# chanzuckerberg/shasta

Hardware: NVIDIA H100
Metric: candidate_pairs_found_and_aligned_per_s (higher is better)
Workload: dtype u64/i32

## Files before the change

shasta_b200/csrc/align.cu:

```cuda
#include "context.cuh"
#include "align_kernels.cuh"
#include "hostpool.cuh"
#include "digest.cuh"

#include <algorithm>
#include <atomic>
#include <exception>
#include <memory>
#include <mutex>
#include <chrono>
#include <cstring>
#include <sys/mman.h>
#include <thread>
#include <limits>
#include <map>
#include <vector>

namespace shb {

extern thread_local uint64_t g_launchCount;

namespace {

uint32_t warpsForClass(const DpClass& k)
{
    if(k.c > 0) return kDpMaxWarpsPerBlock;
    const uint64_t perWarp = 3ull * (k.wMax + 1) * 4;
    const uint32_t w = uint32_t(std::min<uint64_t>(kDpMaxWarpsPerBlock, (200ull * 1024) / perWarp));
    return w ? w : 1;
}
size_t smemForClass(const DpClass& k, uint32_t warps) { return k.c > 0 ? 0 : size_t(warps) * 3 * (k.wMax + 1) * 4; }
size_t scanKernelSmemLimit()
{
    size_t most = 0;
    for(uint32_t k = 0; k < kDpClassCount; k++) most = std::max(most, smemForClass(dpClassAt(k), warpsForClass(dpClassAt(k))));
// ... 207 lines not shown
    const uint32_t rows = uint32_t(2 * c->readCountTotal);
    sc.sortedKmer.reserve(M + 1);
    sc.sortedOrdinal.reserve(M + 1);
    const std::vector<uint64_t>& toc = c->tocHost;
    DeviceBuffer<uint64_t> keysA, keysB;
    DeviceBuffer<uint32_t> valsA, valsB;
    const uint64_t chunkLimit = envCount("SHB_ALIGN4_SORT_CHUNK", 1u << 28);
    uint32_t rowBegin = 0;
    while(rowBegin < rows) {
        uint32_t rowEnd = rowBegin + 1;
        while(rowEnd < rows && toc[rowEnd + 1] - toc[rowBegin] <= chunkLimit) rowEnd++;
        const uint64_t markerBegin = toc[rowBegin];
        const uint64_t n64 = toc[rowEnd] - markerBegin;
        SHB_REQUIRE(n64 < (1ull << 32), SHB_ERR_INVALID, "An oriented read has more than 2^32-1 markers.");
        const uint32_t n = uint32_t(n64);
        if(n) {
            keysA.reserve(n); keysB.reserve(n); valsA.reserve(n); valsB.reserve(n);
            SHB_LAUNCH(sortedMarkerKeysKernel, ceilDiv(n, 256), 256, 0, st, c->kmerIds, (const uint64_t*)c->toc.get(),
                       rowBegin, rowEnd, markerBegin, n, keysA.get(), valsA.get());
            const uint32_t rowBits = bitsFor(rowEnd - rowBegin - 1);
            const int ranges[2][2] = {{0, int(2 * k)}, {32, 32 + int(rowBits)}};
            const bool inB = radixSort<true>(keysA.get(), keysB.get(), valsA.get(), valsB.get(), n, ranges, 2, c->sortWs, st);
            SHB_LAUNCH(sortedMarkerUnpackKernel, ceilDiv(n, 256), 256, 0, st, (const uint64_t*)(inB ? keysB.get() : keysA.get()), n,
                       sc.sortedKmer.get() + markerBegin);
            SHB_CUDA(cudaMemcpyAsync(sc.sortedOrdinal.get() + markerBegin, inB ? valsB.get() : valsA.get(), 4ull * n,
                                     cudaMemcpyDeviceToDevice, st));
        }
        rowBegin = rowEnd;
    }
    SHB_CUDA(cudaStreamSynchronize(st));
    sc.sortedGeneration = c->markerGeneration;
}

void parallelMemcpy(uint8_t* dst, const uint8_t* src, uint64_t n)
{
    constexpr int kThreads = 4;
    if(n < (4ull << 20)) { memcpy(dst, src, n); return; }
    std::thread workers[kThreads - 1];
    const uint64_t part = (n / kThreads + 4095) & ~4095ull;
    for(int t = 1; t < kThreads; t++) {
        const uint64_t off = std::min<uint64_t>(n, part * t), len = std::min<uint64_t>(part, n - off);
        workers[t - 1] = std::thread([=] { if(len) memcpy(dst + off, src + off, len); });
    }
    memcpy(dst, src, std::min<uint64_t>(part, n));
    for(int t = 1; t < kThreads; t++) workers[t - 1].join();
}

void copyToHostPipelined(shb_context* c, void* dstHost, const void* srcDevice, uint64_t bytes, bool pageLocked)
{
    if(bytes == 0) return;
    if(pageLocked) {
        SHB_CUDA(cudaMemcpyAsync(dstHost, srcDevice, bytes, cudaMemcpyDeviceToHost, c->stream));
        return;
    }
    constexpr uint64_t kChunk = 32ull << 20;
    if(!c->pinnedStage[0]) {
        SHB_CUDA(cudaHostAlloc(&c->pinnedStage[0], kChunk, cudaHostAllocDefault));
        SHB_CUDA(cudaHostAlloc(&c->pinnedStage[1], kChunk, cudaHostAllocDefault));
        SHB_CUDA(cudaEventCreateWithFlags(&c->stageEvent[0], cudaEventDisableTiming));
        SHB_CUDA(cudaEventCreateWithFlags(&c->stageEvent[1], cudaEventDisableTiming));
    }
    cudaStream_t st = c->stream;
    const uint64_t chunks = (bytes + kChunk - 1) / kChunk;
    for(uint64_t k = 0; k <= chunks; k++) {
        if(k < chunks) {
            const uint64_t off = k * kChunk, n = std::min(kChunk, bytes - off);
            SHB_CUDA(cudaMemcpyAsync(c->pinnedStage[k & 1], static_cast<const uint8_t*>(srcDevice) + off, n, cudaMemcpyDeviceToHost, st));
            SHB_CUDA(cudaEventRecord(c->stageEvent[k & 1], st));
        }
        if(k > 0) {
            const uint64_t j = k - 1, off = j * kChunk, n = std::min(kChunk, bytes - off);
            SHB_CUDA(cudaEventSynchronize(c->stageEvent[j & 1]));
            parallelMemcpy(static_cast<uint8_t*>(dstHost) + off, static_cast<const uint8_t*>(c->pinnedStage[j & 1]), n);
        }
    }
}

void buildClassOrder(AlignWorker& w, const DpJob* jobs, uint32_t nJobs, std::vector<uint64_t>& classCounts, bool forward = false)
{
    cudaStream_t st = w.stream;
    Batch& b = w.batch;
    classCounts.assign(kDpClassCount + (forward ? kDpForwardClassCount : 0), 0);
    if(nJobs == 0) return;
    b.orderKeysA.reserve(nJobs); b.orderKeysB.reserve(nJobs); b.orderValsA.reserve(nJobs); b.orderValsB.reserve(nJobs);
    SHB_LAUNCH(dpClassKeysKernel, ceilDiv(nJobs, 256), 256, 0, st, jobs, nJobs, forward, b.orderKeysA.get(), b.orderValsA.get());
    const int ranges[1][2] = {{0, kDpLengthKeyBits + kDpClassKeyBits}};
    const bool inB = radixSort<true>(b.orderKeysA.get(), b.orderKeysB.get(), b.orderValsA.get(), b.orderValsB.get(), nJobs, ranges, 1, w.sortWs, st);
    b.order = inB ? b.orderValsB.get() : b.orderValsA.get();
    unsigned long long* dCounts = w.sc(kScDigits);
    SHB_CUDA(cudaMemsetAsync(dCounts, 0, 256 * sizeof(unsigned long long), st));
    SHB_LAUNCH(digitCountKernel, ceilDiv(nJobs, 256), 256, 0, st, (const uint64_t*)(inB ? b.orderKeysB.get() : b.orderKeysA.get()), nJobs, kDpLengthKeyBits, kDpClassNone, dCounts);
    unsigned long long h[256];
    SHB_CUDA(cudaMemcpyAsync(h, dCounts, sizeof(h), cudaMemcpyDeviceToHost, st));
    SHB_CUDA(cudaStreamSynchronize(st));
    for(size_t k = 0; k < classCounts.size(); k++) classCounts[k] = h[k];
}

template<class F> void runDpClasses(AlignWorker& w, const std::vector<uint64_t>& classCounts, uint32_t chunkMax, uint32_t firstBanded,
                                    const DpJob* jobs, const uint32_t* sequences, DpScores scores, F launchOther)
{
    Batch& b = w.batch;
    BandedArgs g;
    g.kmerIds = sequences; g.scores = scores; g.fma = FmaUnits{1, 2, 4};
    size_t unit = 0;
    forEachClassConcurrently(w, classCounts, chunkMax, [&](int k, uint32_t count, uint64_t offset, cudaStream_t s) {
        const uint32_t* order = b.order + offset;
        if(uint32_t(k) < firstBanded) { launchOther(uint32_t(k), count, order, s); return; }
        const uint32_t cls = uint32_t(k) - firstBanded;
        BandedArgs gk = g;
        gk.n = count; gk.order = order; gk.wMax = dpClassAt(cls).wMax;
// ... 33 lines not shown
    b.ordinals.reserve(ordinalSlots + 1);
    b.runs.reserve(ordinalSlots + 1);
    w.traceWords += traceWords;
    SHB_LAUNCH(setTraceOffsetsKernel, ceilDiv(nJobs, 256), 256, 0, st, b.jobs.get(), nJobs, (const unsigned long long*)b.twOff.get(),
               (const unsigned long long*)b.outOff.get());
    SHB_LAUNCH(bandCellsKernel, ceilDiv(nJobs, 256), 256, 0, st, (const DpJob*)b.jobs.get(), nJobs, w.sc(kScBandCells));
    SHB_CUDA(cudaMemsetAsync(b.counts.get(), 0, 4ull * nJobs, st));
    std::vector<uint64_t> classCounts;
    buildClassOrder(w, b.jobs.get(), nJobs, classCounts);
    SHB_CUDA(cudaEventRecord(w.dp2a, st));
    runDpClasses(w, classCounts, envCount("SHB_ALIGN_CHUNK", 32768), 0, b.jobs.get(), sequences, scores,
                 [](uint32_t, uint32_t, const uint32_t*, cudaStream_t) {});
    SHB_CUDA(cudaEventRecord(w.dp2b, st));
}

struct AlignCall {
    shb_context* c;
    AlignCache* ac;
    const uint32_t* cand; uint64_t n;
    shb_align_options o;
    bool method4;
    DpScores scores; FilterOptions fo;
    uint32_t batchMax;
    uint32_t align4SmemCells = kAlign4SmemCells;
    std::mutex dispenserMutex;
    uint64_t nextBegin = 0, nextIndex = 0;
    struct Segment { uint64_t recordBase = 0, kept = 0, byteBase = 0, bytes = 0; };
    std::mutex arenaMutex;
    std::map<uint64_t, Segment> ledger;
    uint64_t outCount = 0, outBytes = 0;
    cudaStream_t finalStream = nullptr;
    unsigned long long* digests = nullptr;
    uint64_t nextToFinalise = 0, finalRecords = 0, finalBytes = 0;
    uint8_t* hostRecords = nullptr; uint8_t* hostToc = nullptr; uint8_t* hostData = nullptr;
    uint64_t hostDataCapacity = 0;
    bool dataOverflow = false;
    std::atomic<bool> failed{false};
    std::exception_ptr error;
    std::mutex errorMutex;
};

bool nextBatch(AlignCall& call, uint64_t& begin, uint32_t& nb, uint64_t& index)
{
    std::lock_guard<std::mutex> lock(call.dispenserMutex);
    if(call.nextBegin >= call.n || call.failed.load()) return false;
    begin = call.nextBegin;
    nb = 0;
    if(call.method4) {
        const std::vector<uint64_t>& toc = call.c->tocHost;
        const uint64_t cellBudget = 768ull << 20;
        uint64_t cells = 0;
        while(begin + nb < call.n && nb < call.batchMax) {
            const uint64_t i = begin + nb;
            const uint64_t o0 = 2ull * call.cand[3*i], o1 = 2ull * call.cand[3*i+1] + ((call.cand[3*i+2] & 0xff) ? 0 : 1);
            const uint64_t nx = toc[o0+1] - toc[o0], ny = toc[o1+1] - toc[o1];
            uint64_t cc = 2;
            if(nx && ny) cc += ((nx + ny - 2) / call.o.align4DeltaX + 1) * ((nx + ny - 2) / call.o.align4DeltaY + 1);
            if(nb && cells + cc > cellBudget) break;
            cells += cc; nb++;
        }
    } else nb = uint32_t(std::min<uint64_t>(call.batchMax, call.n - begin));
    index = call.nextIndex++;
    call.nextBegin += nb;
    return true;
}

__global__ void rebaseTocKernel(unsigned long long* __restrict__ toc, uint64_t n, long long delta)
{
    const uint64_t i = uint64_t(blockIdx.x) * blockDim.x + threadIdx.x;
    if(i < n) toc[i] = (unsigned long long)((long long)toc[i] + delta);
}

void finaliseReadySegments(AlignCall& call)
{
    AlignCache& ac = *call.ac;
    cudaStream_t fs = call.finalStream;
    for(;;) {
        auto it = call.ledger.find(call.nextToFinalise);
        if(it == call.ledger.end()) break;
        const AlignCall::Segment& seg = it->second;
        if(seg.kept) {
            unsigned long long* segToc = ac.outToc.get() + seg.recordBase;
            const long long delta = (long long)call.finalBytes - (long long)seg.byteBase;
            if(delta) SHB_LAUNCH(rebaseTocKernel, ceilDiv(seg.kept, 256), 256, 0, fs, segToc, seg.kept, delta);
            SHB_LAUNCH(digestRecordsKernel, ceilDiv(seg.kept, 256), 256, 0, fs, (const uint32_t*)ac.outRecords.get() + 16 * seg.recordBase,
                       seg.kept, 16u, call.digests);
            SHB_LAUNCH(digestCompressedKernel, ceilDiv(seg.kept, 256), 256, 0, fs, (const uint32_t*)ac.outRecords.get() + 16 * seg.recordBase,
                       seg.kept, (const unsigned long long*)segToc, call.finalBytes + seg.bytes,
                       (const uint8_t*)ac.outData.get() + seg.byteBase - call.finalBytes, call.digests + 1);
            if(call.hostRecords) {
                SHB_CUDA(cudaMemcpyAsync(call.hostRecords + 64 * call.finalRecords, ac.outRecords.get() + 16 * seg.recordBase, 64 * seg.kept, cudaMemcpyDeviceToHost, fs));
                SHB_CUDA(cudaMemcpyAsync(call.hostToc + 8 * call.finalRecords, segToc, 8 * seg.kept, cudaMemcpyDeviceToHost, fs));
                if(!call.dataOverflow && call.finalBytes + seg.bytes <= call.hostDataCapacity) {
                    SHB_CUDA(cudaMemcpyAsync(call.hostData + call.finalBytes, ac.outData.get() + seg.byteBase, seg.bytes, cudaMemcpyDeviceToHost, fs));
                } else call.dataOverflow = true;
            }
            call.finalRecords += seg.kept; call.finalBytes += seg.bytes;
        }
        call.nextToFinalise++;
    }
}

void processBatch(AlignCall& call, AlignWorker& w, uint64_t begin, uint32_t nb, uint64_t batchIndex)
{
    shb_context* c = call.c;
    AlignCache& ac = *call.ac;
    const shb_align_options& o = call.o;
    cudaStream_t st = w.stream;
    Batch& b = w.batch;
    unsigned long long* total64 = w.sc(kScTotal64);
    uint32_t* total32 = reinterpret_cast<uint32_t*>(w.sc(kScTotal32));

    b.cand.reserve(3ull * nb);
    SHB_CUDA(cudaMemcpyAsync(b.cand.get(), call.cand + 3 * begin, 12ull * nb, cudaMemcpyHostToDevice, st));
    b.keep.reserve(nb); b.keepIndex.reserve(nb); b.bytes32.reserve(nb); b.bytes64.reserve(nb); b.bytesOff.reserve(nb);
    b.scanWs64.reserve(scanWorkspaceElements(nb));
    w.scanWs.reserve(scanWorkspaceElements(std::max<uint64_t>(nb, 4096)));
    uint32_t nJobs = 0;
    const uint32_t* jobIndex = nullptr;
    bool stage1Timed = false;

    if(!call.method4) {
        const bool method1 = (o.alignMethod == 1);
        nJobs = nb;
        b.jobs1.reserve(nb); b.jobs.reserve(nb); b.tw.reserve(nb); b.twOff.reserve(nb); b.outCnt.reserve(nb);
        SHB_LAUNCH(method3SetupKernel, ceilDiv(nb, 256), 256, 0, st, (const uint32_t*)b.cand.get(), nb,
                   (const uint64_t*)c->toc.get(), method1 ? (const uint64_t*)nullptr : (const uint64_t*)ac.dsToc.get(), b.jobs1.get(), b.jobs.get(),
                   b.tw.get(), b.outCnt.get(), w.sc(kScForwardCells), kMaxBandWidth, w.sc(kScTooWide));
        if(!method1) {
// ... 216 lines not shown
                    longest = std::max<uint64_t>(longest, c->tocHost[o + 1] - c->tocHost[o]);
                }
            }
            SHB_REQUIRE(fits(longest), SHB_ERR_INVALID,
                        "Align scores too large for the reads: max(|matchScore|, |mismatchScore|, |gapScore|) * "
                        "(2 * longest read in markers + 16384) must be below 2^28.");
        }
    }
    if(call.method4) {
        SHB_REQUIRE(o.align4DeltaX >= 1 && o.align4DeltaY >= 1 && o.align4DeltaX < (1ull << 31) && o.align4DeltaY < (1ull << 31),
                    SHB_ERR_INVALID, "Invalid Align.align4.deltaX / deltaY.");
        buildSortedMarkers(c, o.k);
    } else if(o.alignMethod == 3) {
        buildDownsampled(c, o.k, o.downsamplingFactor);
    }
    const uint32_t maxStage2Width = uint32_t(std::max(0, o.maxBand)) + 3 + 64;
    SHB_REQUIRE(maxStage2Width <= kMaxBandWidth, SHB_ERR_INVALID, "Align.maxBand too large for this implementation (limit 16317).");

    call.fo.minAlignedMarkerCount = uint64_t(o.minAlignedMarkerCount); call.fo.maxSkip = uint64_t(o.maxSkip);
    call.fo.maxDrift = uint64_t(o.maxDrift); call.fo.maxTrim = uint64_t(o.maxTrim);
    call.fo.minAlignedFraction = o.minAlignedFraction;
    call.fo.suppressContainments = (!call.method4 && o.suppressContainments) ? 1u : 0u;

    call.batchMax = envCount("SHB_ALIGN_BATCH", call.method4 ? 32768 : (o.alignMethod == 1 ? 16384 : 262144));
    call.align4SmemCells = std::min<uint32_t>(kAlign4SmemCells, envCount("SHB_ALIGN4_SMEM_CELLS", kAlign4SmemCells));
    const uint64_t batchEstimate = (n + call.batchMax - 1) / call.batchMax;
    const uint32_t workerCount = uint32_t(std::max<uint64_t>(1, std::min<uint64_t>(envCount("SHB_ALIGN_WORKERS", 2), batchEstimate)));
    while(ac.workers.size() < workerCount) ac.workers.emplace_back(new AlignWorker());
    for(uint32_t k = 0; k < workerCount; k++) ac.workers[k]->init();
    if(!ac.finalStream) SHB_CUDA(cudaStreamCreateWithFlags(&ac.finalStream, cudaStreamNonBlocking));
    call.finalStream = ac.finalStream;
    call.digests = c->scalar(kSlotAlignmentDigests);
    SHB_CUDA(cudaMemsetAsync(call.digests, 0, 2 * sizeof(unsigned long long), st));
    HostResult recOut, tocOut, dataOut;
    if(n && ac.lastBytesPerCandidate > 0.) {
        const uint64_t dataEstimate = uint64_t(ac.lastBytesPerCandidate * double(n) * 1.03) + (1ull << 20);
        recOut.reset(allocHostResult(64 * n)); tocOut.reset(allocHostResult(8 * (n + 1))); dataOut.reset(allocHostResult(dataEstimate));
        if(recOut.p && tocOut.p && dataOut.p && HostPool::instance().isPageLocked(recOut.p) && HostPool::instance().isPageLocked(tocOut.p) &&
           HostPool::instance().isPageLocked(dataOut.p)) {
            call.hostRecords = static_cast<uint8_t*>(recOut.p); call.hostToc = static_cast<uint8_t*>(tocOut.p);
            call.hostData = static_cast<uint8_t*>(dataOut.p); call.hostDataCapacity = dataEstimate;
        }
    }
    SHB_CUDA(cudaStreamSynchronize(st));

    if(n) {
        std::vector<std::thread> threads;
        for(uint32_t k = 0; k < workerCount; k++) threads.emplace_back([&call, &ac, k] { workerMain(call, *ac.workers[k]); });
        for(std::thread& t : threads) t.join();
        if(call.error) std::rethrow_exception(call.error);
    }

    SHB_CUDA(cudaStreamSynchronize(call.finalStream));
    const uint64_t count = call.outCount, outBytes = call.outBytes;
    const auto copy0 = std::chrono::steady_clock::now();
    SHB_REQUIRE(call.nextToFinalise == call.ledger.size() && call.finalRecords == count && call.finalBytes == outBytes, SHB_ERR_CUDA,
                "Internal error: not every batch was finalised.");
    const bool earlyCopy = call.hostRecords != nullptr;
    if(!earlyCopy) {
        recOut.reset(allocHostResult(64 * count)); tocOut.reset(allocHostResult(8 * (count + 1)));
    }
    if(!earlyCopy || call.dataOverflow) dataOut.reset(allocHostResult(outBytes));
    SHB_REQUIRE(recOut.p && tocOut.p && dataOut.p, SHB_ERR_OOM, "Out of host memory for the alignments.");
    if(count && (!earlyCopy || call.dataOverflow)) {
        const bool lockedRec = HostPool::instance().isPageLocked(recOut.p), lockedToc = HostPool::instance().isPageLocked(tocOut.p),
                   lockedData = HostPool::instance().isPageLocked(dataOut.p);
        uint64_t finalRecords = 0, finalBytes = 0;
        for(const auto& entry : call.ledger) {
            const AlignCall::Segment& seg = entry.second;
            if(!seg.kept) continue;
            if(!earlyCopy) {
                copyToHostPipelined(c, static_cast<uint8_t*>(recOut.p) + 64 * finalRecords, ac.outRecords.get() + 16 * seg.recordBase, 64 * seg.kept, lockedRec);
                copyToHostPipelined(c, static_cast<uint8_t*>(tocOut.p) + 8 * finalRecords, ac.outToc.get() + seg.recordBase, 8 * seg.kept, lockedToc);
            }
            copyToHostPipelined(c, static_cast<uint8_t*>(dataOut.p) + finalBytes, ac.outData.get() + seg.byteBase, seg.bytes, lockedData);
            finalRecords += seg.kept; finalBytes += seg.bytes;
        }
        SHB_CUDA(cudaStreamSynchronize(st));
    }
    if(n) ac.lastBytesPerCandidate = double(outBytes) / double(n);
    unsigned long long* digests = call.digests;
    unsigned long long skipped = 0, forwardCells = 0, tooWide = 0, bandCells = 0, digestHost[2] = {0, 0};
    uint64_t traceWords = 0, launches = g_launchCount;
    double dpMs = 0.;
    for(uint32_t k = 0; k < workerCount && n; k++) {
        AlignWorker& w = *ac.workers[k];
        unsigned long long h[6];
        SHB_CUDA(cudaMemcpyAsync(h, w.scalars.get(), sizeof(h), cudaMemcpyDeviceToHost, st));
        SHB_CUDA(cudaStreamSynchronize(st));
        skipped += h[kScSkipped]; forwardCells += h[kScForwardCells]; tooWide += h[kScTooWide]; bandCells += h[kScBandCells];
        traceWords += w.traceWords; launches += w.launches; dpMs += w.dpMs;
    }
    SHB_CUDA(cudaMemcpyAsync(digestHost, digests, sizeof(digestHost), cudaMemcpyDeviceToHost, st));
    SHB_CUDA(cudaStreamSynchronize(st));
    uint64_t* tocHostOut = static_cast<uint64_t*>(tocOut.p);
    tocHostOut[count] = outBytes;
    if(count == 0) tocHostOut[0] = 0;
    totalTimer.stop(st);
    SHB_CUDA(cudaStreamSynchronize(st));
    const float totalMs = totalTimer.elapsedMs();
    if(getenv("SHB_TRACE")) {
        fprintf(stderr, "[shb] computeAlignments: %u worker(s), %llu batches, %llu candidates skipped as too wide for the DP kernels\n",
                workerCount, (unsigned long long)call.ledger.size(), tooWide);
    }
    if(result) {
        memset(result, 0, sizeof(*result));
        result->candidateCount = n; result->alignmentCount = count; result->skippedCount = skipped;
        result->dpCells = 16ull * traceWords + forwardCells;
        result->dpUsefulCells = bandCells + forwardCells;
        result->tooWideCount = tooWide;
        result->dpMs = dpMs / double(workerCount); result->totalMs = totalMs; result->kernelLaunches = launches;
        result->alignmentDataDigest = digestHost[0]; result->compressedDigest = digestHost[1];
        result->workers = workerCount;
        result->outputCopyMs = msSince(copy0);
        result->hostWallMs = msSince(wall0);
    }
    *alignmentDataOut = recOut.take(); *alignmentCountOut = count;
    *compressedTocOut = static_cast<uint64_t*>(tocOut.take()); *compressedDataOut = static_cast<uint8_t*>(dataOut.take());
}

}
```

shasta_b200/csrc/api.cu:

```cuda
#include "context.cuh"
#include <vector>
#include "lowhash_kernels.cuh"
#include "hostpool.cuh"
#include "digest.cuh"

#include <cstring>
#include <string>

namespace shb {

static thread_local std::string g_lastError;
void setLastError(const std::string& message) { g_lastError = message; }

void lowhash0(shb_context* c, const shb_lowhash_params& p, void** candidatesOut, uint64_t* candidateCountOut,
              uint64_t* statsOut, uint64_t* iterSummary, uint64_t maxIterSummary, shb_lowhash_result* result);

void computeAlignments(shb_context* c, const void* candidatesHost, uint64_t n, const shb_align_options& o,
                       void** alignmentDataOut, uint64_t* alignmentCountOut,
                       uint64_t** compressedTocOut, uint8_t** compressedDataOut, shb_align_result* result,
                       bool explicitOrientation);
void destroyAlignCache(shb_context* c);
void destroyLowhashState(shb_context* c);
void destroyDistState(shb_context* c);
LowHashState& lowhashState(shb_context* c);
// ... 85 lines not shown

const char* shb_last_error(void) { return g_lastError.c_str(); }

shb_status shb_context_create(int device, shb_context** ctx)
{
    return guarded([&] {
        SHB_REQUIRE(ctx != nullptr, SHB_ERR_INVALID, "Null context pointer.");
        int count = 0;
        SHB_CUDA(cudaGetDeviceCount(&count));
        SHB_REQUIRE(device >= 0 && device < count, SHB_ERR_CUDA, "No such CUDA device.");
        cudaDeviceProp prop;
        SHB_CUDA(cudaGetDeviceProperties(&prop, device));
        SHB_REQUIRE(prop.major == 9 && prop.minor == 0, SHB_ERR_CUDA,
                    std::string("shasta_b200 is built for sm_90a (H100) only; device is sm_") + std::to_string(prop.major) + std::to_string(prop.minor));
        SHB_CUDA(cudaSetDevice(device));
        shb_context* c = new shb_context();
        c->device = device;
        SHB_CUDA(cudaStreamCreateWithFlags(&c->stream, cudaStreamNonBlocking));
        SHB_CUDA(cudaStreamCreateWithFlags(&c->copyStream[0], cudaStreamNonBlocking));
        SHB_CUDA(cudaStreamCreateWithFlags(&c->copyStream[1], cudaStreamNonBlocking));
        c->scalars.reserve(shb::kScalarWords);
        *ctx = c;
    });
}

void shb_context_destroy(shb_context* c)
{
    if(!c) return;
    cudaSetDevice(c->device);
    cudaDeviceSynchronize();
    destroyDistState(c);
    destroyAlignCache(c);
    destroyLowhashState(c);
    for(int i = 0; i < 2; i++) { if(c->pinnedStage[i]) cudaFreeHost(c->pinnedStage[i]); if(c->stageEvent[i]) cudaEventDestroy(c->stageEvent[i]); }
    if(c->stream) cudaStreamDestroy(c->stream);
    for(int i = 0; i < 2; i++) if(c->copyStream[i]) cudaStreamDestroy(c->copyStream[i]);
    delete c;
}

void shb_free(void* p) { shb::HostPool::instance().release(p); }
void shb_trim_host_cache(void) { shb::HostPool::instance().trim(); }

shb_status shb_set_markers(shb_context* c, uint64_t readCountTotal, uint64_t readBegin, uint64_t readEnd,
                           const uint64_t* toc, const uint8_t* markerData7, const uint8_t* readFlags,
                           uint64_t totalMarkerCount)
{
    return guarded([&] {
        SHB_REQUIRE(c != nullptr, SHB_ERR_INVALID, "Null context.");
        SHB_CUDA(cudaSetDevice(c->device));
        c->haveMarkers = false;
        setCommonMarkerState(c, readCountTotal, readBegin, readEnd, toc, readFlags, totalMarkerCount);
        const uint64_t M = c->localMarkerCount;
        SHB_REQUIRE(markerData7 != nullptr || M == 0, SHB_ERR_INVALID, "Null marker data.");
        c->kmerIdsOwned.reserve(M + 64);
        const uint64_t chunkMarkers = (uint64_t(envCount("SHB_MARKER_UPLOAD_CHUNK", 32u << 20)) + 1023) & ~1023ull;
        const uint64_t chunkBytes = chunkMarkers * 7;
        DeviceBuffer<uint8_t> staging[2];
        for(uint64_t begin = 0, k = 0; begin < M; begin += chunkMarkers, k++) {
            const int b = int(k & 1);
            const uint64_t nMarkers = std::min(chunkMarkers, M - begin);
            const uint64_t nBytes = nMarkers * 7;
            if(!staging[b].get()) staging[b].reserve(std::min(chunkBytes, M * 7) + 16);
            cudaStream_t s = c->copyStream[b];
            SHB_CUDA(cudaMemcpyAsync(staging[b].get(), markerData7 + begin * 7, nBytes, cudaMemcpyHostToDevice, s));
            const uint64_t wordCount = (nBytes + 3) / 4;
            SHB_LAUNCH(extractKmerIdsKernel, ceilDiv(nMarkers, kExtractMarkersPerBlock), kExtractThreads, 0, s,
                       reinterpret_cast<const uint32_t*>(staging[b].get()), wordCount, nMarkers,
// ... 429 lines not shown
```

shasta_b200/csrc/context.cuh:

```cuda
#pragma once

#include "common.cuh"
#include "primitives.cuh"

#include <cstdlib>
#include <vector>

namespace shb {
inline uint32_t envCount(const char* name, uint32_t dflt)
{
    const char* v = std::getenv(name);
    if(!v) return dflt;
    const long x = std::strtol(v, nullptr, 10);
    return x > 0 ? uint32_t(x) : dflt;
}

constexpr int kMaxFusedIterations = 16;

enum ScalarSlot : uint32_t {
    kSlotSweepCounts = 0,
    kSlotSegmentTotal = kSlotSweepCounts + kMaxFusedIterations,
    kSlotPairCursor,
    kSlotPairHits,
    kSlotCandidateDigest,
    kSlotPartitionCounts,
    kSlotDownsampleTotal = kSlotPartitionCounts + 256,
    kSlotAlignmentDigests,
    kSlotMarkerTotal = kSlotAlignmentDigests + 2,
    kSlotKeptAlignments,
    kSlotBadConnectivity,
    kSlotMarkerGraphVertices,
    kSlotMarkerGraphRcErrors = kSlotMarkerGraphVertices + 6,
    kSlotMarkerGraphEdges = kSlotMarkerGraphRcErrors + 2,
    kSlotMarkerGraphRcEdges = kSlotMarkerGraphEdges + 8,
    kScalarSlotEnd = kSlotMarkerGraphRcEdges + 4
};
constexpr uint32_t kScalarWords = 512;
static_assert(kScalarSlotEnd <= kScalarWords, "the scalar slots do not fit the reserved words");

struct Footprint {
    uint64_t live = 0, peak = 0;
    template<class T> void add(DeviceBuffer<T>& b, uint64_t n)
    {
        const uint64_t before = b.capacity();
        b.reserve(n);
        live += (b.capacity() - before) * sizeof(T);
        peak = std::max(peak, live);
    }
    template<class T> void drop(DeviceBuffer<T>& b) { live -= b.capacity() * sizeof(T); b.release(); }
};
// ... 25 lines not shown
    cudaStream_t copyStream[2] = {nullptr, nullptr};

    bool haveMarkers = false;
    uint64_t markerGeneration = 0;
    uint64_t readCountTotal = 0;
    uint64_t readBegin = 0, readEnd = 0;
    uint64_t totalMarkerCount = 0;
    uint64_t localMarkerCount = 0;
    shb::DeviceBuffer<uint32_t> kmerIdsOwned;
    const uint32_t* kmerIds = nullptr;
    shb::DeviceBuffer<uint64_t> toc;
    shb::DeviceBuffer<uint8_t> readFlags;
    std::vector<uint64_t> tocHost;
    std::vector<uint8_t> readFlagsHost;

    shb::SortWorkspace sortWs;
    shb::DeviceBuffer<uint32_t> scanWs;
    shb::DeviceBuffer<unsigned long long> scalars;
    unsigned long long* scalar(shb::ScalarSlot slot) const { return scalars.get() + slot; }

    shb::DeviceBuffer<uint64_t> sweepKeys;  shb::DeviceBuffer<uint32_t> sweepVals;
    shb::DeviceBuffer<uint32_t> sweepTileFirstRead;
    uint64_t sweepTileGeneration = ~0ull;
    shb::DeviceBuffer<uint64_t> entryKeysTmp; shb::DeviceBuffer<uint32_t> entryValsTmp;
    shb::DeviceBuffer<uint32_t> flagsBuf, indexBuf, segStartBuf, countsBuf;
    shb::DeviceBuffer<uint64_t> pairsA, pairsB;
    shb::DeviceBuffer<uint64_t> accKeysA, accKeysB;
    shb::DeviceBuffer<uint32_t> accValsA, accValsB;
    shb::DeviceBuffer<unsigned long long> stats;
    shb::DeviceBuffer<uint32_t> candidatesDev;

    shb::DeviceBuffer<uint64_t> partKeys; shb::DeviceBuffer<uint32_t> partVals;
    void* lowhashState = nullptr;
    void* pinnedStage[2] = {nullptr, nullptr};
    cudaEvent_t stageEvent[2] = {nullptr, nullptr};

    void* alignCache = nullptr;
    void* dist = nullptr;
};

namespace shb {
inline void requireWholeAssembly(shb_context* c, const char* what)
{
    SHB_REQUIRE(c->haveMarkers, SHB_ERR_STATE, "No markers: call shb_set_markers* or shb_find_markers first.");
    SHB_REQUIRE(c->readBegin == 0 && c->readEnd == c->readCountTotal, SHB_ERR_STATE,
                std::string(what) + " needs the markers of every read on one context.");
}
}
```

shasta_b200/csrc/hostpool.cuh:

```cuda
#pragma once
#include <cstdint>
#include <cstdlib>
#include <mutex>
#include <unordered_map>
#include <vector>
#include <sys/mman.h>
#include <cuda_runtime.h>

namespace shb {

class HostPool {
public:
    static HostPool& instance()
    {
        static HostPool* pool = new HostPool();
        return *pool;
    }

    void* allocate(uint64_t bytes)
    {
        if(bytes < kLargeBytes) return malloc(bytes ? bytes : 1);
        std::lock_guard<std::mutex> lock(mutex_);
        int best = -1;
        for(size_t k = 0; k < free_.size(); k++) {
            if(free_[k].capacity >= bytes && free_[k].capacity / 4 <= bytes && (best < 0 || free_[k].capacity < free_[size_t(best)].capacity)) best = int(k);
        }
        Block blk;
        if(best >= 0) {
            blk = free_[size_t(best)];
            free_.erase(free_.begin() + best);
            if(!blk.registered && !blk.registerFailed) {
                if(cudaHostRegister(blk.p, blk.capacity, cudaHostRegisterPortable) == cudaSuccess) blk.registered = true;
                else { cudaGetLastError(); blk.registerFailed = true; }
            }
        } else {
            const uint64_t slack = bytes + bytes / 8;
            blk.capacity = (slack + kAlign - 1) & ~(kAlign - 1);
            void* p = nullptr;
            if(posix_memalign(&p, kAlign, blk.capacity) != 0) return nullptr;
            madvise(p, blk.capacity, MADV_HUGEPAGE);
            blk.p = p;
        }
        live_[blk.p] = blk;
        return blk.p;
    }

    void release(void* p)
    {
        if(!p) return;
        std::lock_guard<std::mutex> lock(mutex_);
        auto it = live_.find(p);
        if(it == live_.end()) { free(p); return; }
        free_.push_back(it->second);
        live_.erase(it);
        while(free_.size() > kMaxCached) { destroy(free_.front()); free_.erase(free_.begin()); }
    }

    bool isPageLocked(const void* p)
    {
        std::lock_guard<std::mutex> lock(mutex_);
        auto it = live_.find(const_cast<void*>(p));
        return it != live_.end() && it->second.registered;
    }

    void trim()
    {
        std::lock_guard<std::mutex> lock(mutex_);
        for(Block& b : free_) destroy(b);
        free_.clear();
    }

private:
    struct Block { void* p = nullptr; uint64_t capacity = 0; bool registered = false, registerFailed = false; };
    static constexpr uint64_t kLargeBytes = 8ull << 20, kAlign = 2ull << 20;
    static constexpr size_t kMaxCached = 8;
    static void destroy(Block& b)
    {
        if(b.registered) { if(cudaHostUnregister(b.p) != cudaSuccess) cudaGetLastError(); }
        free(b.p);
    }
    std::mutex mutex_;
    std::vector<Block> free_;
    std::unordered_map<void*, Block> live_;
};

inline void* allocHostResult(uint64_t bytes) { return HostPool::instance().allocate(bytes); }

struct HostResult {
    void* p = nullptr;
    explicit HostResult(void* q = nullptr) : p(q) {}
    HostResult(const HostResult&) = delete;
    HostResult& operator=(const HostResult&) = delete;
    ~HostResult() { if(p) HostPool::instance().release(p); }
    void* take() { void* q = p; p = nullptr; return q; }
    void reset(void* q) { if(p) HostPool::instance().release(p); p = q; }
};

}
```

shasta_b200/csrc/lowhash.cu:

```cuda
#include "context.cuh"
#include "lowhash_kernels.cuh"
#include "hostpool.cuh"
#include "digest.cuh"

#include <algorithm>
#include <cmath>
#include <cstring>
#include <limits>
#include <vector>

namespace shb {

thread_local uint64_t g_launchCount = 0;

namespace {

const uint32_t kUnrolledGroups[] = {16, 10, 8, 4, 2, 1};

uint32_t nextSweepGroupImpl(uint64_t remaining, uint64_t slabCapacity)
{
    constexpr uint64_t kSlabBudgetBytes = 16ull << 30;
    const uint64_t fit = std::max<uint64_t>(1, kSlabBudgetBytes / (12ull * std::max<uint64_t>(slabCapacity, 1)));
    for(uint32_t g : kUnrolledGroups) if(g <= remaining && g <= fit) return g;
    return 1;
}

template<int MM, int KK> void launchSweepKernel(const SweepArgs& a, uint32_t blocks, cudaStream_t stream)
{
    const size_t dynamicBytes = size_t(a.queueCapacity) * 16;
    static size_t allowed = 0;
    if(dynamicBytes > allowed) {
        SHB_CUDA(cudaFuncSetAttribute(lowhashSweepKernel<MM, KK>, cudaFuncAttributeMaxDynamicSharedMemorySize, int(dynamicBytes)));
        allowed = dynamicBytes;
    }
    SHB_LAUNCH((lowhashSweepKernel<MM, KK>), blocks, kSweepThreads, dynamicBytes, stream, a);
// ... 367 lines not shown
                   (const uint32_t*)c->flagsBuf.get(), (const uint32_t*)c->indexBuf.get(), uint32_t(S.acc.count),
                   c->candidatesDev.get());
        SHB_LAUNCH(digestRecordsKernel, ceilDiv(nOut, 256), 256, 0, st, (const uint32_t*)c->candidatesDev.get(), nOut, 3u, digestDev);
    }
    S.emittedCount = nOut;
    return nOut;
}

void lowhashReleaseLargeScratch(shb_context* c)
{
    auto bytes = [](auto& b) { return uint64_t(b.capacity()) * sizeof(*b.get()); };
    const uint64_t total = bytes(c->pairsA) + bytes(c->pairsB) + bytes(c->flagsBuf) + bytes(c->indexBuf) + bytes(c->segStartBuf) +
                           bytes(c->countsBuf) + bytes(c->scanWs) + bytes(c->accKeysA) + bytes(c->accKeysB) + bytes(c->accValsA) +
                           bytes(c->accValsB) + bytes(c->entryKeysTmp) + bytes(c->entryValsTmp) + bytes(c->sweepKeys) +
                           bytes(c->sweepVals) + bytes(c->partKeys) + bytes(c->partVals);
    if(total < (32ull << 30)) return;
    SHB_CUDA(cudaStreamSynchronize(c->stream));
    c->pairsA.release(); c->pairsB.release(); c->flagsBuf.release(); c->indexBuf.release(); c->segStartBuf.release();
    c->countsBuf.release(); c->scanWs.release(); c->accKeysA.release(); c->accKeysB.release(); c->accValsA.release();
    c->accValsB.release(); c->entryKeysTmp.release(); c->entryValsTmp.release(); c->sweepKeys.release(); c->sweepVals.release();
    c->partKeys.release(); c->partVals.release();
    c->sortWs.status.release();
    LowHashState& S = lowhashState(c);
    const uint64_t rawLimit = S.acc.rawLimit;
    S.acc = LowHashAccumulator();
    S.acc.rawLimit = rawLimit;
}

void lowhashEmit(shb_context* c, void** candidatesOut, uint64_t* candidateCountOut)
{
    LowHashState& S = lowhashState(c);
    const uint64_t nOut = lowhashEmitDevice(c);
    cudaStream_t st = c->stream;
    HostResult host(allocHostResult(nOut * 12));
    SHB_REQUIRE(host.p != nullptr, SHB_ERR_OOM, "Out of host memory for the alignment candidates.");
    unsigned long long digest = 0;
    if(nOut) SHB_CUDA(cudaMemcpyAsync(host.p, c->candidatesDev.get(), nOut * 12, cudaMemcpyDeviceToHost, st));
    SHB_CUDA(cudaMemcpyAsync(&digest, c->scalar(kSlotCandidateDigest), sizeof(digest), cudaMemcpyDeviceToHost, st));
    SHB_CUDA(cudaStreamSynchronize(st));
    S.candidateDigest = digest;
    *candidatesOut = host.take();
    *candidateCountOut = nOut;
}

void devicePartition(shb_context* c, uint64_t* keys, uint32_t* vals, uint64_t n, uint32_t shift, uint32_t bits,
                     uint64_t* counts, uint64_t** keysOut, uint32_t** valsOut)
{
    SHB_REQUIRE(bits <= 8 && shift + bits <= 64, SHB_ERR_INVALID, "Invalid partition digit.");
    SHB_REQUIRE(n < (1ull << 32), SHB_ERR_INVALID, "Too many items to partition.");
    SHB_CUDA(cudaSetDevice(c->device));
    cudaStream_t st = c->stream;
    const uint32_t buckets = 1u << bits;
    for(uint32_t d = 0; d < buckets; d++) counts[d] = 0;
    if(n == 0 || bits == 0) {
        if(bits == 0) counts[0] = n;
        *keysOut = keys; *valsOut = vals;
        return;
    }
    c->partKeys.reserve(n);
    c->partVals.reserve(n);
    const int range[1][2] = {{int(shift), int(shift + bits)}};
    const bool inB = radixSort<true>(keys, c->partKeys.get(), vals, c->partVals.get(), n, range, 1, c->sortWs, st);
    uint64_t* sortedKeys = inB ? c->partKeys.get() : keys;
    unsigned long long* dCounts = c->scalar(kSlotPartitionCounts);
    SHB_CUDA(cudaMemsetAsync(dCounts, 0, buckets * sizeof(unsigned long long), st));
    SHB_LAUNCH(digitCountKernel, ceilDiv(n, 256), 256, 0, st, (const uint64_t*)sortedKeys, uint32_t(n), int(shift), buckets - 1u, dCounts);
    std::vector<unsigned long long> h(buckets);
    SHB_CUDA(cudaMemcpyAsync(h.data(), dCounts, buckets * sizeof(unsigned long long), cudaMemcpyDeviceToHost, st));
    SHB_CUDA(cudaStreamSynchronize(st));
    for(uint32_t d = 0; d < buckets; d++) counts[d] = h[d];
    *keysOut = sortedKeys;
    *valsOut = inB ? c->partVals.get() : vals;
}

// ... 75 lines not shown
```

Measured before the change: 11.25 million.

## Stream alignment results to host through a threaded pinned staging ring

Replaces the end-of-call pipelined device-to-host copy with a StagedCopier. Its worker threads stage each finalised segment through an 8-slot pinned ring while later batches are still aligning, so the output copy overlaps compute even when the host result buffers are not page-locked. Host blocks are now mmap-backed and can grow with mremap when the data estimate is exceeded, instead of falling back to a full recopy. The candidate emit path also uses the copier. This adds threads, locking on the arena mutex, and more complex buffer-growth logic.

```diff
diff --git a/shasta_b200/csrc/align.cu b/shasta_b200/csrc/align.cu
--- a/shasta_b200/csrc/align.cu
+++ b/shasta_b200/csrc/align.cu
@@ -1,6 +1,6 @@
 #include "context.cuh"
 #include "align_kernels.cuh"
-#include "hostpool.cuh"
+#include "hostcopy.cuh"
 #include "digest.cuh"
 
 #include <algorithm>
@@ -274,50 +274,6 @@
     sc.sortedGeneration = c->markerGeneration;
 }
 
-void parallelMemcpy(uint8_t* dst, const uint8_t* src, uint64_t n)
-{
-    constexpr int kThreads = 4;
-    if(n < (4ull << 20)) { memcpy(dst, src, n); return; }
-    std::thread workers[kThreads - 1];
-    const uint64_t part = (n / kThreads + 4095) & ~4095ull;
-    for(int t = 1; t < kThreads; t++) {
-        const uint64_t off = std::min<uint64_t>(n, part * t), len = std::min<uint64_t>(part, n - off);
-        workers[t - 1] = std::thread([=] { if(len) memcpy(dst + off, src + off, len); });
-    }
-    memcpy(dst, src, std::min<uint64_t>(part, n));
-    for(int t = 1; t < kThreads; t++) workers[t - 1].join();
-}
-
-void copyToHostPipelined(shb_context* c, void* dstHost, const void* srcDevice, uint64_t bytes, bool pageLocked)
-{
-    if(bytes == 0) return;
-    if(pageLocked) {
-        SHB_CUDA(cudaMemcpyAsync(dstHost, srcDevice, bytes, cudaMemcpyDeviceToHost, c->stream));
-        return;
-    }
-    constexpr uint64_t kChunk = 32ull << 20;
-    if(!c->pinnedStage[0]) {
-        SHB_CUDA(cudaHostAlloc(&c->pinnedStage[0], kChunk, cudaHostAllocDefault));
-        SHB_CUDA(cudaHostAlloc(&c->pinnedStage[1], kChunk, cudaHostAllocDefault));
-        SHB_CUDA(cudaEventCreateWithFlags(&c->stageEvent[0], cudaEventDisableTiming));
-        SHB_CUDA(cudaEventCreateWithFlags(&c->stageEvent[1], cudaEventDisableTiming));
-    }
-    cudaStream_t st = c->stream;
-    const uint64_t chunks = (bytes + kChunk - 1) / kChunk;
-    for(uint64_t k = 0; k <= chunks; k++) {
-        if(k < chunks) {
-            const uint64_t off = k * kChunk, n = std::min(kChunk, bytes - off);
-            SHB_CUDA(cudaMemcpyAsync(c->pinnedStage[k & 1], static_cast<const uint8_t*>(srcDevice) + off, n, cudaMemcpyDeviceToHost, st));
-            SHB_CUDA(cudaEventRecord(c->stageEvent[k & 1], st));
-        }
-        if(k > 0) {
-            const uint64_t j = k - 1, off = j * kChunk, n = std::min(kChunk, bytes - off);
-            SHB_CUDA(cudaEventSynchronize(c->stageEvent[j & 1]));
-            parallelMemcpy(static_cast<uint8_t*>(dstHost) + off, static_cast<const uint8_t*>(c->pinnedStage[j & 1]), n);
-        }
-    }
-}
-
 void buildClassOrder(AlignWorker& w, const DpJob* jobs, uint32_t nJobs, std::vector<uint64_t>& classCounts, bool forward = false)
 {
     cudaStream_t st = w.stream;
@@ -417,9 +373,10 @@
     cudaStream_t finalStream = nullptr;
     unsigned long long* digests = nullptr;
     uint64_t nextToFinalise = 0, finalRecords = 0, finalBytes = 0;
-    uint8_t* hostRecords = nullptr; uint8_t* hostToc = nullptr; uint8_t* hostData = nullptr;
-    uint64_t hostDataCapacity = 0;
-    bool dataOverflow = false;
+    HostBlock* hostRecords = nullptr; HostBlock* hostToc = nullptr; HostBlock* hostData = nullptr;
+    StagedCopier* copier = nullptr;
+    bool dataDirect = false;
+    uint64_t dataDirectCapacity = 0;
     std::atomic<bool> failed{false};
     std::exception_ptr error;
     std::mutex errorMutex;
@@ -473,13 +430,21 @@
             SHB_LAUNCH(digestCompressedKernel, ceilDiv(seg.kept, 256), 256, 0, fs, (const uint32_t*)ac.outRecords.get() + 16 * seg.recordBase,
                        seg.kept, (const unsigned long long*)segToc, call.finalBytes + seg.bytes,
                        (const uint8_t*)ac.outData.get() + seg.byteBase - call.finalBytes, call.digests + 1);
-            if(call.hostRecords) {
-                SHB_CUDA(cudaMemcpyAsync(call.hostRecords + 64 * call.finalRecords, ac.outRecords.get() + 16 * seg.recordBase, 64 * seg.kept, cudaMemcpyDeviceToHost, fs));
-                SHB_CUDA(cudaMemcpyAsync(call.hostToc + 8 * call.finalRecords, segToc, 8 * seg.kept, cudaMemcpyDeviceToHost, fs));
-                if(!call.dataOverflow && call.finalBytes + seg.bytes <= call.hostDataCapacity) {
-                    SHB_CUDA(cudaMemcpyAsync(call.hostData + call.finalBytes, ac.outData.get() + seg.byteBase, seg.bytes, cudaMemcpyDeviceToHost, fs));
-                } else call.dataOverflow = true;
-            }
+            const AlignCache* acp = &ac;
+            const uint64_t recordBase = seg.recordBase, byteBase = seg.byteBase;
+            if(call.hostRecords->pageLocked) {
+                SHB_CUDA(cudaMemcpyAsync(call.hostRecords->data() + 64 * call.finalRecords, ac.outRecords.get() + 16 * seg.recordBase, 64 * seg.kept, cudaMemcpyDeviceToHost, fs));
+            } else call.copier->copy(*call.hostRecords, 64 * call.finalRecords,
+                                     [acp, recordBase] { return reinterpret_cast<const uint8_t*>(acp->outRecords.get() + 16 * recordBase); }, 64 * seg.kept);
+            if(call.hostToc->pageLocked) {
+                SHB_CUDA(cudaMemcpyAsync(call.hostToc->data() + 8 * call.finalRecords, segToc, 8 * seg.kept, cudaMemcpyDeviceToHost, fs));
+            } else call.copier->copy(*call.hostToc, 8 * call.finalRecords,
+                                     [acp, recordBase] { return reinterpret_cast<const uint8_t*>(acp->outToc.get() + recordBase); }, 8 * seg.kept);
+            if(call.dataDirect && call.finalBytes + seg.bytes > call.dataDirectCapacity) call.dataDirect = false;
+            if(call.dataDirect) {
+                SHB_CUDA(cudaMemcpyAsync(call.hostData->data() + call.finalBytes, ac.outData.get() + seg.byteBase, seg.bytes, cudaMemcpyDeviceToHost, fs));
+            } else call.copier->copy(*call.hostData, call.finalBytes,
+                                     [acp, byteBase] { return acp->outData.get() + byteBase; }, seg.bytes);
             call.finalRecords += seg.kept; call.finalBytes += seg.bytes;
         }
         call.nextToFinalise++;
@@ -762,16 +727,11 @@
     call.finalStream = ac.finalStream;
     call.digests = c->scalar(kSlotAlignmentDigests);
     SHB_CUDA(cudaMemsetAsync(call.digests, 0, 2 * sizeof(unsigned long long), st));
-    HostResult recOut, tocOut, dataOut;
-    if(n && ac.lastBytesPerCandidate > 0.) {
-        const uint64_t dataEstimate = uint64_t(ac.lastBytesPerCandidate * double(n) * 1.03) + (1ull << 20);
-        recOut.reset(allocHostResult(64 * n)); tocOut.reset(allocHostResult(8 * (n + 1))); dataOut.reset(allocHostResult(dataEstimate));
-        if(recOut.p && tocOut.p && dataOut.p && HostPool::instance().isPageLocked(recOut.p) && HostPool::instance().isPageLocked(tocOut.p) &&
-           HostPool::instance().isPageLocked(dataOut.p)) {
-            call.hostRecords = static_cast<uint8_t*>(recOut.p); call.hostToc = static_cast<uint8_t*>(tocOut.p);
-            call.hostData = static_cast<uint8_t*>(dataOut.p); call.hostDataCapacity = dataEstimate;
-        }
-    }
+    const uint64_t dataEstimate = n ? uint64_t((ac.lastBytesPerCandidate > 0. ? ac.lastBytesPerCandidate * 1.03 : 64.) * double(n)) + (1ull << 20) : 0;
+    HostBlock recOut(64 * n), tocOut(8 * (n + 1)), dataOut(dataEstimate);
+    StagedCopier copier(c, call.finalStream, 4, &call.arenaMutex);
+    call.hostRecords = &recOut; call.hostToc = &tocOut; call.hostData = &dataOut; call.copier = &copier;
+    call.dataDirect = dataOut.pageLocked; call.dataDirectCapacity = dataEstimate;
     SHB_CUDA(cudaStreamSynchronize(st));
 
     if(n) {
@@ -781,33 +741,12 @@
         if(call.error) std::rethrow_exception(call.error);
     }
 
+    const auto copy0 = std::chrono::steady_clock::now();
     SHB_CUDA(cudaStreamSynchronize(call.finalStream));
+    copier.finish();
     const uint64_t count = call.outCount, outBytes = call.outBytes;
-    const auto copy0 = std::chrono::steady_clock::now();
     SHB_REQUIRE(call.nextToFinalise == call.ledger.size() && call.finalRecords == count && call.finalBytes == outBytes, SHB_ERR_CUDA,
                 "Internal error: not every batch was finalised.");
-    const bool earlyCopy = call.hostRecords != nullptr;
-    if(!earlyCopy) {
-        recOut.reset(allocHostResult(64 * count)); tocOut.reset(allocHostResult(8 * (count + 1)));
-    }
-    if(!earlyCopy || call.dataOverflow) dataOut.reset(allocHostResult(outBytes));
-    SHB_REQUIRE(recOut.p && tocOut.p && dataOut.p, SHB_ERR_OOM, "Out of host memory for the alignments.");
-    if(count && (!earlyCopy || call.dataOverflow)) {
-        const bool lockedRec = HostPool::instance().isPageLocked(recOut.p), lockedToc = HostPool::instance().isPageLocked(tocOut.p),
-                   lockedData = HostPool::instance().isPageLocked(dataOut.p);
-        uint64_t finalRecords = 0, finalBytes = 0;
-        for(const auto& entry : call.ledger) {
-            const AlignCall::Segment& seg = entry.second;
-            if(!seg.kept) continue;
-            if(!earlyCopy) {
-                copyToHostPipelined(c, static_cast<uint8_t*>(recOut.p) + 64 * finalRecords, ac.outRecords.get() + 16 * seg.recordBase, 64 * seg.kept, lockedRec);
-                copyToHostPipelined(c, static_cast<uint8_t*>(tocOut.p) + 8 * finalRecords, ac.outToc.get() + seg.recordBase, 8 * seg.kept, lockedToc);
-            }
-            copyToHostPipelined(c, static_cast<uint8_t*>(dataOut.p) + finalBytes, ac.outData.get() + seg.byteBase, seg.bytes, lockedData);
-            finalRecords += seg.kept; finalBytes += seg.bytes;
-        }
-        SHB_CUDA(cudaStreamSynchronize(st));
-    }
     if(n) ac.lastBytesPerCandidate = double(outBytes) / double(n);
     unsigned long long* digests = call.digests;
     unsigned long long skipped = 0, forwardCells = 0, tooWide = 0, bandCells = 0, digestHost[2] = {0, 0};
@@ -823,7 +762,7 @@
     }
     SHB_CUDA(cudaMemcpyAsync(digestHost, digests, sizeof(digestHost), cudaMemcpyDeviceToHost, st));
     SHB_CUDA(cudaStreamSynchronize(st));
-    uint64_t* tocHostOut = static_cast<uint64_t*>(tocOut.p);
+    uint64_t* tocHostOut = reinterpret_cast<uint64_t*>(tocOut.data());
     tocHostOut[count] = outBytes;
     if(count == 0) tocHostOut[0] = 0;
     totalTimer.stop(st);
@@ -845,8 +784,8 @@
         result->outputCopyMs = msSince(copy0);
         result->hostWallMs = msSince(wall0);
     }
-    *alignmentDataOut = recOut.take(); *alignmentCountOut = count;
-    *compressedTocOut = static_cast<uint64_t*>(tocOut.take()); *compressedDataOut = static_cast<uint8_t*>(dataOut.take());
-}
-
-}
+    *alignmentDataOut = recOut.owner.take(); *alignmentCountOut = count;
+    *compressedTocOut = static_cast<uint64_t*>(tocOut.owner.take()); *compressedDataOut = static_cast<uint8_t*>(dataOut.owner.take());
+}
+
+}
diff --git a/shasta_b200/csrc/api.cu b/shasta_b200/csrc/api.cu
--- a/shasta_b200/csrc/api.cu
+++ b/shasta_b200/csrc/api.cu
@@ -141,7 +141,7 @@
     destroyDistState(c);
     destroyAlignCache(c);
     destroyLowhashState(c);
-    for(int i = 0; i < 2; i++) { if(c->pinnedStage[i]) cudaFreeHost(c->pinnedStage[i]); if(c->stageEvent[i]) cudaEventDestroy(c->stageEvent[i]); }
+    for(int i = 0; i < shb::kStageSlots; i++) { if(c->pinnedStage[i]) cudaFreeHost(c->pinnedStage[i]); if(c->stageEvent[i]) cudaEventDestroy(c->stageEvent[i]); }
     if(c->stream) cudaStreamDestroy(c->stream);
     for(int i = 0; i < 2; i++) if(c->copyStream[i]) cudaStreamDestroy(c->copyStream[i]);
     delete c;
diff --git a/shasta_b200/csrc/context.cuh b/shasta_b200/csrc/context.cuh
--- a/shasta_b200/csrc/context.cuh
+++ b/shasta_b200/csrc/context.cuh
@@ -16,6 +16,8 @@
 }
 
 constexpr int kMaxFusedIterations = 16;
+constexpr int kStageSlots = 8;
+constexpr uint64_t kStageBytes = 8ull << 20;
 
 enum ScalarSlot : uint32_t {
     kSlotSweepCounts = 0,
@@ -107,8 +109,8 @@
 
     shb::DeviceBuffer<uint64_t> partKeys; shb::DeviceBuffer<uint32_t> partVals;
     void* lowhashState = nullptr;
-    void* pinnedStage[2] = {nullptr, nullptr};
-    cudaEvent_t stageEvent[2] = {nullptr, nullptr};
+    void* pinnedStage[shb::kStageSlots] = {};
+    cudaEvent_t stageEvent[shb::kStageSlots] = {};
 
     void* alignCache = nullptr;
     void* dist = nullptr;
diff --git a/shasta_b200/csrc/hostcopy.cuh b/shasta_b200/csrc/hostcopy.cuh
--- /dev/null
+++ b/shasta_b200/csrc/hostcopy.cuh
@@ -0,0 +1,167 @@
+#pragma once
+#include "context.cuh"
+#include "hostpool.cuh"
+
+#include <condition_variable>
+#include <deque>
+#include <exception>
+#include <functional>
+#include <mutex>
+#include <shared_mutex>
+#include <thread>
+#include <vector>
+
+namespace shb {
+
+struct HostBlock {
+    HostResult owner;
+    uint64_t capacity = 0;
+    bool pageLocked = false;
+    std::shared_mutex resize;
+    explicit HostBlock(uint64_t bytes) : owner(allocHostResult(bytes)), capacity(bytes)
+    {
+        SHB_REQUIRE(owner.p != nullptr, SHB_ERR_OOM, "Out of host memory for the results.");
+        pageLocked = HostPool::instance().isPageLocked(owner.p);
+    }
+    uint8_t* data() const { return static_cast<uint8_t*>(owner.p); }
+};
+
+inline void ensureStagingRing(shb_context* c)
+{
+    if(c->pinnedStage[0]) return;
+    for(int i = 0; i < kStageSlots; i++) {
+        SHB_CUDA(cudaHostAlloc(&c->pinnedStage[i], kStageBytes, cudaHostAllocDefault));
+        SHB_CUDA(cudaEventCreateWithFlags(&c->stageEvent[i], cudaEventDisableTiming));
+    }
+}
+
+class StagedCopier {
+public:
+    StagedCopier(shb_context* c, cudaStream_t stream, int threads, std::mutex* srcLock = nullptr)
+        : c_(c), stream_(stream), srcLock_(srcLock)
+    {
+        SHB_REQUIRE(threads >= 1 && 2 * threads <= kStageSlots, SHB_ERR_INVALID, "Too many copier threads for the staging ring.");
+        ensureStagingRing(c);
+        for(int t = 0; t < threads; t++) threads_.emplace_back([this, t] { run(t); });
+    }
+    StagedCopier(const StagedCopier&) = delete;
+    StagedCopier& operator=(const StagedCopier&) = delete;
+    ~StagedCopier() { stop(); }
+
+    void copy(HostBlock& dst, uint64_t dstOffset, std::function<const uint8_t*()> src, uint64_t bytes)
+    {
+        if(bytes == 0) return;
+        std::lock_guard<std::mutex> lock(mutex_);
+        for(uint64_t off = 0; off < bytes; off += kStageBytes) {
+            const uint64_t n = std::min<uint64_t>(kStageBytes, bytes - off);
+            pieces_.push_back(Piece{&dst, dstOffset + off, src, off, n});
+        }
+        ready_.notify_all();
+    }
+
+    void finish()
+    {
+        stop();
+        if(error_) std::rethrow_exception(error_);
+    }
+
+private:
+    struct Piece { HostBlock* dst; uint64_t dstOffset; std::function<const uint8_t*()> src; uint64_t srcOffset, bytes; };
+
+    void stop()
+    {
+        {
+            std::lock_guard<std::mutex> lock(mutex_);
+            done_ = true;
+        }
+        ready_.notify_all();
+        for(std::thread& t : threads_) if(t.joinable()) t.join();
+        threads_.clear();
+    }
+
+    bool take(Piece& p, bool wait)
+    {
+        std::unique_lock<std::mutex> lock(mutex_);
+        if(wait) ready_.wait(lock, [this] { return !pieces_.empty() || done_ || failed_; });
+        if(pieces_.empty() || failed_) return false;
+        p = std::move(pieces_.front());
+        pieces_.pop_front();
+        return true;
+    }
+
+    void issue(const Piece& p, int slot)
+    {
+        {
+            std::unique_lock<std::mutex> lock;
+            if(srcLock_) lock = std::unique_lock<std::mutex>(*srcLock_);
+            SHB_CUDA(cudaMemcpyAsync(c_->pinnedStage[slot], p.src() + p.srcOffset, p.bytes, cudaMemcpyDeviceToHost, stream_));
+        }
+        SHB_CUDA(cudaEventRecord(c_->stageEvent[slot], stream_));
+    }
+
+    void drain(const Piece& p, int slot)
+    {
+        SHB_CUDA(cudaEventSynchronize(c_->stageEvent[slot]));
+        HostBlock& b = *p.dst;
+        const uint64_t end = p.dstOffset + p.bytes;
+        std::shared_lock<std::shared_mutex> shared(b.resize);
+        if(end > b.capacity) {
+            shared.unlock();
+            {
+                std::unique_lock<std::shared_mutex> exclusive(b.resize);
+                if(end > b.capacity) {
+                    const uint64_t capacity = std::max(end, b.capacity + b.capacity / 2);
+                    void* q = HostPool::instance().grow(b.owner.p, b.capacity, capacity);
+                    SHB_REQUIRE(q != nullptr, SHB_ERR_OOM, "Out of host memory for the results.");
+                    b.owner.p = q; b.capacity = capacity; b.pageLocked = false;
+                }
+            }
+            shared.lock();
+        }
+        memcpy(b.data() + p.dstOffset, c_->pinnedStage[slot], p.bytes);
+    }
+
+    void run(int t)
+    {
+        try {
+            SHB_CUDA(cudaSetDevice(c_->device));
+            Piece cur, next;
+            int k = 0;
+            bool haveCur = take(cur, true);
+            if(haveCur) issue(cur, 2 * t);
+            while(haveCur) {
+                const bool haveNext = take(next, false);
+                if(haveNext) issue(next, 2 * t + ((k + 1) & 1));
+                drain(cur, 2 * t + (k & 1));
+                k++;
+                if(haveNext) cur = std::move(next);
+                else if((haveCur = take(cur, true))) issue(cur, 2 * t + (k & 1));
+            }
+        } catch(...) {
+            std::lock_guard<std::mutex> lock(mutex_);
+            if(!error_) error_ = std::current_exception();
+            failed_ = true;
+            ready_.notify_all();
+        }
+    }
+
+    shb_context* c_;
+    cudaStream_t stream_;
+    std::mutex* srcLock_;
+    std::mutex mutex_;
+    std::condition_variable ready_;
+    std::deque<Piece> pieces_;
+    bool done_ = false, failed_ = false;
+    std::exception_ptr error_;
+    std::vector<std::thread> threads_;
+};
+
+inline void copyResult(StagedCopier& copier, cudaStream_t stream, HostBlock& dst, uint64_t dstOffset, const uint8_t* src, uint64_t bytes)
+{
+    if(bytes == 0) return;
+    if(dst.pageLocked && dstOffset + bytes <= dst.capacity) {
+        SHB_CUDA(cudaMemcpyAsync(dst.data() + dstOffset, src, bytes, cudaMemcpyDeviceToHost, stream));
+    } else copier.copy(dst, dstOffset, [src] { return src; }, bytes);
+}
+
+}
diff --git a/shasta_b200/csrc/hostpool.cuh b/shasta_b200/csrc/hostpool.cuh
--- a/shasta_b200/csrc/hostpool.cuh
+++ b/shasta_b200/csrc/hostpool.cuh
@@ -1,6 +1,7 @@
 #pragma once
 #include <cstdint>
 #include <cstdlib>
+#include <cstring>
 #include <mutex>
 #include <unordered_map>
 #include <vector>
@@ -36,13 +37,39 @@
         } else {
             const uint64_t slack = bytes + bytes / 8;
             blk.capacity = (slack + kAlign - 1) & ~(kAlign - 1);
-            void* p = nullptr;
-            if(posix_memalign(&p, kAlign, blk.capacity) != 0) return nullptr;
-            madvise(p, blk.capacity, MADV_HUGEPAGE);
-            blk.p = p;
+            blk.p = mapAligned(blk.capacity);
+            if(!blk.p) return nullptr;
         }
         live_[blk.p] = blk;
         return blk.p;
+    }
+
+    void* grow(void* p, uint64_t used, uint64_t bytes)
+    {
+        std::unique_lock<std::mutex> lock(mutex_);
+        auto it = live_.find(p);
+        if(it == live_.end()) {
+            lock.unlock();
+            void* q = allocate(bytes);
+            if(q) { memcpy(q, p, used); free(p); }
+            return q;
+        }
+        Block blk = it->second;
+        if(blk.capacity >= bytes) return p;
+        const uint64_t capacity = (bytes + bytes / 8 + kAlign - 1) & ~(kAlign - 1);
+        void* q = mapAligned(capacity);
+        if(!q) return nullptr;
+        if(blk.registered && cudaHostUnregister(blk.p) != cudaSuccess) cudaGetLastError();
+        it->second.registered = false;
+        if(mremap(blk.p, blk.capacity, capacity, MREMAP_MAYMOVE | MREMAP_FIXED, q) == MAP_FAILED) {
+            munmap(q, capacity);
+            return nullptr;
+        }
+        madvise(q, capacity, MADV_HUGEPAGE);
+        live_.erase(it);
+        blk.p = q; blk.capacity = capacity; blk.registered = false;
+        live_[q] = blk;
+        return q;
     }
 
     void release(void* p)
@@ -74,10 +101,20 @@
     struct Block { void* p = nullptr; uint64_t capacity = 0; bool registered = false, registerFailed = false; };
     static constexpr uint64_t kLargeBytes = 8ull << 20, kAlign = 2ull << 20;
     static constexpr size_t kMaxCached = 8;
+    static void* mapAligned(uint64_t bytes)
+    {
+        void* raw = mmap(nullptr, bytes + kAlign, PROT_READ | PROT_WRITE, MAP_PRIVATE | MAP_ANONYMOUS, -1, 0);
+        if(raw == MAP_FAILED) return nullptr;
+        const uintptr_t r = reinterpret_cast<uintptr_t>(raw), a = (r + kAlign - 1) & ~(kAlign - 1);
+        if(a > r) munmap(raw, a - r);
+        if(r + kAlign > a) munmap(reinterpret_cast<void*>(a + bytes), r + kAlign - a);
+        madvise(reinterpret_cast<void*>(a), bytes, MADV_HUGEPAGE);
+        return reinterpret_cast<void*>(a);
+    }
     static void destroy(Block& b)
     {
         if(b.registered) { if(cudaHostUnregister(b.p) != cudaSuccess) cudaGetLastError(); }
-        free(b.p);
+        munmap(b.p, b.capacity);
     }
     std::mutex mutex_;
     std::vector<Block> free_;
diff --git a/shasta_b200/csrc/lowhash.cu b/shasta_b200/csrc/lowhash.cu
--- a/shasta_b200/csrc/lowhash.cu
+++ b/shasta_b200/csrc/lowhash.cu
@@ -1,6 +1,6 @@
 #include "context.cuh"
 #include "lowhash_kernels.cuh"
-#include "hostpool.cuh"
+#include "hostcopy.cuh"
 #include "digest.cuh"
 
 #include <algorithm>
@@ -434,14 +434,17 @@
     LowHashState& S = lowhashState(c);
     const uint64_t nOut = lowhashEmitDevice(c);
     cudaStream_t st = c->stream;
-    HostResult host(allocHostResult(nOut * 12));
-    SHB_REQUIRE(host.p != nullptr, SHB_ERR_OOM, "Out of host memory for the alignment candidates.");
+    HostBlock host(nOut * 12);
     unsigned long long digest = 0;
-    if(nOut) SHB_CUDA(cudaMemcpyAsync(host.p, c->candidatesDev.get(), nOut * 12, cudaMemcpyDeviceToHost, st));
-    SHB_CUDA(cudaMemcpyAsync(&digest, c->scalar(kSlotCandidateDigest), sizeof(digest), cudaMemcpyDeviceToHost, st));
-    SHB_CUDA(cudaStreamSynchronize(st));
+    {
+        StagedCopier copier(c, st, 3);
+        copyResult(copier, st, host, 0, reinterpret_cast<const uint8_t*>(c->candidatesDev.get()), nOut * 12);
+        SHB_CUDA(cudaMemcpyAsync(&digest, c->scalar(kSlotCandidateDigest), sizeof(digest), cudaMemcpyDeviceToHost, st));
+        SHB_CUDA(cudaStreamSynchronize(st));
+        copier.finish();
+    }
     S.candidateDigest = digest;
-    *candidatesOut = host.take();
+    *candidatesOut = host.owner.take();
     *candidateCountOut = nOut;
 }
 
```

Measured after the change: 12.09 million (median of 6 runs). 1.07x the previous value.
